# zjwzcx/A-2D-LiDAR-based-SLAM-System-for-Wheeled-Mobile-Robots

Measured on AMD Instinct MI355X. Metric: scans/sec (360-beam ICP + 0.05 m grid update), higher is better.
Workload: dtype f64; 1 GPU; configs[1]: 1000-scan replay (every 5th message of a 10 Hz stream, seed 1), 360 beams, ICP(max_iter=30, tol=0.001) + 400x400@0.05m grid, f64 point buffers; 32 independent replays of the 1000-scan trajectory per step (one slam_replay_dev call: ranges [32, 1000, 360], a map per trajectory); point_buffers=f64, pipeline=0, lanes=2, grid_mode=1, grid_group=16, parallelism=1 trajectory per GPU (32 independent replays of it per step)

## Files before the change

a-2d-lidar-based-slam-system-for-wheeled-mobile-robots_amd/csrc/icp_kernels.hip:

```cpp
#include <hip/hip_fp16.h>
#include <hip/hip_runtime.h>

#include <type_traits>

#include "slam_internal.h"
#include "slam_stamps.h"

namespace slam {

#ifdef SLAM_STAMPS_ICP
__device__ unsigned long long g_polar_lanes[4];
hipError_t debug_polar_lanes(unsigned long long out[4], bool clear)
{
    hipError_t e = hipMemcpyFromSymbol(out, HIP_SYMBOL(g_polar_lanes), sizeof(unsigned long long) * 4);
    if (e == hipSuccess && clear) {
        const unsigned long long zero[4] = {0ull, 0ull, 0ull, 0ull};
        e = hipMemcpyToSymbol(HIP_SYMBOL(g_polar_lanes), zero, sizeof zero);
    }
    return e;
}
#endif

__device__ __forceinline__ double ld(const double *p, long i) { return p[i]; }
__device__ __forceinline__ double ld(const float *p, long i) { return (double)p[i]; }
__device__ __forceinline__ double ld(const __half *p, long i) { return (double)__half2float(p[i]); }
__device__ __forceinline__ void st(double *p, long i, double v) { p[i] = v; }
__device__ __forceinline__ void st(float *p, long i, double v) { p[i] = (float)v; }
__device__ __forceinline__ void st(__half *p, long i, double v)
{
    float f = (float)v;
    if ((double)f != v && v == v) {
// ... 284 lines not shown
constexpr int kPolarMaxFirst = 16;
constexpr int kPolarMaxListed = 48;
constexpr int kPolarProbe = 8;
constexpr bool kOnePass = true;
constexpr int kPolarTail = 4;

template <typename T> struct StoreSlack { static constexpr float ang = 2e-7f; };
template <> struct StoreSlack<float> { static constexpr float ang = 1e-6f; };
template <> struct StoreSlack<__half> { static constexpr float ang = 3e-3f; };

struct PolarGeo {
    float inv_db;
    float slack;
};

template <int UNROLL, bool PROBE>
__device__ __forceinline__ void nn_polar(const double2 *__restrict__ tarP, int n_tar, double sx, double sy, int seed,
                                         bool active, const PolarGeo &geo, int wmax, double &best_d2, int &best_j, bool &big,
                                         bool &amb, unsigned long long &ambm)
{
    const float fsx = (float)sx, fsy = (float)sy;
    const float rs2 = fsx * fsx + fsy * fsy;
    int lo, hi;
    auto window = [&](int j, int &wlo, int &whi) -> bool {
        const double2 ts = tarP[j];
        const double U = dist2(sx, sy, ts.x, ts.y);
        const float ftx = (float)ts.x, fty = (float)ts.y;
        const float x2 = ((float)U * 1.000002f + 1e-30f) * __builtin_amdgcn_rcpf(rs2 * 0.999998f);
        const bool small = x2 < 0.25f;
        const float x = __builtin_amdgcn_sqrtf(x2) * 1.000001f;
        const float alpha = x * (1.0f + 0.19f * x2) * 1.000002f + geo.slack;
        const float y = (ftx * fsy - fty * fsx) * __builtin_amdgcn_rcpf(ftx * fsx + fty * fsy);
        const float y3 = y * y * y * 0.33333334f;
        const float dhi = (y >= 0.0f ? y : y - y3) + 4e-6f;
// ... 37 lines not shown
        pb.start();
        pb.j = seed;
        scan(need ? max(seed - kPolarProbe, 0) : 1, need ? min(seed + kPolarProbe, n_tar - 1) : 0, pb);
        int lo1, hi1;
        const bool fits1 = window(pb.j, lo1, hi1) && need;
        lo = fits1 ? lo1 : lo;
        hi = fits1 ? hi1 : hi;
        fits = fits || fits1;
    }
    big = active && !fits;
    const bool go = active && !big;
    const int m0 = max(lo, 0), m1 = min(hi, n_tar - 1);
    Best b;
    b.start();
    const bool wraps = __any(go && ((hi >= n_tar - 2 && lo >= 1) || (lo <= 1 && hi <= n_tar - 2)));
    if (wraps) {
        const int e0 = hi >= n_tar - 2 ? min(hi - (n_tar - 1) + 1, m0 - 1) : -1;
        scan(go ? 0 : 1, go ? e0 : 0, b);
    }
    scan(go ? m0 : 1, go ? m1 : 0, b);
    if (wraps) {
        const int s2 = lo <= 1 ? max(n_tar - 1 + lo - 1, m1 + 1) : n_tar;
        scan(go ? s2 : 1, go ? n_tar - 1 : 0, b);
    }
    best_d2 = b.d2;
    best_j = b.j;
    amb = go && b.amb();
    ambm = b.ambm;
}

// ... 265 lines not shown
    PolarGeo pg;
    pg.inv_db = polar ? __fdividef(1.000002f, dmin) : 0.0f;
    pg.slack = StoreSlack<T>::ang;
    return pg;
}

struct NNTarget {
    const double2 *tarP;
    const double2 *tarB;
    const Box *boxes, *boxes4;
    int nblocks, n_tar;
    bool has_p;
    double2 *qlist;
    int *qseed;
    int cap;
    __device__ __forceinline__ double2 at(int j) const { return has_p ? tarP[j] : tarB[tslot(j)]; }
};
struct NNQuery {
    double d2;
    int j;
    int slot;
};
__device__ __forceinline__ double match_distance(double d2) { return (d2 < INFINITY) ? sqrt(d2) : 0.0; }

template <int UNROLL, int STRIDE, bool EXACT, typename Place, typename NoteBig>
__device__ __forceinline__ NNQuery nn_query(const NNTarget &t, const PolarGeo &pg, const double sx, const double sy, const int seed, const bool okq,
                                            const bool first, const bool listing, Place &&place, NoteBig &&note_big, unsigned long long &amb_mask)
{
    NNQuery h;
    h.slot = -1;
    if (EXACT) {
        const bool padded = STRIDE == kNNStride && !t.has_p;
        const NNHit e = nn_exact(padded ? t.tarB : t.tarP, padded, okq ? t.n_tar : 0, sx, sy);
        h.d2 = e.d2; h.j = e.j;
    } else if (pg.inv_db > 0.0f) {
        bool big, amb_lane;
        unsigned long long am;
        nn_polar<UNROLL, false>(t.tarP, t.n_tar, sx, sy, seed, okq, pg, listing ? kPolarMaxFirst : kPolarMax, h.d2, h.j, big, amb_lane, am);
        (void)amb_lane;
        amb_mask |= am;
        if (listing) {
            const unsigned long long bm = __ballot(big);
            if (bm != 0ull) {
                const int pos = place(bm) + (int)__builtin_amdgcn_mbcnt_hi((unsigned)(bm >> 32), __builtin_amdgcn_mbcnt_lo((unsigned)bm, 0u));
                if (big && pos < t.cap) {
                    h.slot = pos;
                    t.qlist[pos] = make_double2(sx, sy);
                    t.qseed[pos] = seed;
                    big = false;
                }
            }
        }
        note_big(big);
// ... 361 lines not shown
    }
    if (tid == 0) store_result(a, b, r, s);
    ISTAMP(5);
    ISTAMP_END(s.iters);
    lds_guard_check(guard, a.status);
    return !EXACT && (nwaves > 1 ? geo[5] != 0u : amb_mask != 0ull);
}

constexpr int kWaveQpt = 6;
constexpr int kWaveRound = 4 * 1024;
__host__ __device__ inline int icp_wave_points(int n_tar)
{
    const int whole = nn_blocks(n_tar) * kNNBlock, tail = n_tar + kPolarTail;
    return whole > tail ? whole : tail;
}
__host__ __device__ inline size_t icp_wave_lds_bytes(int n_tar, int cap)
{
    return (size_t)icp_wave_points(n_tar) * sizeof(double2) + (size_t)(nn_boxes_padded(n_tar) + nn_boxes4(n_tar)) * sizeof(Box) +
           (size_t)cap * (sizeof(double2) + sizeof(int));
}

__device__ __forceinline__ double sqrt_unscaled(double x)
{
    const double y = __builtin_amdgcn_rsq(x);
    double g = x * y, h = y * 0.5;
    const double r = fma(-h, g, 0.5);
    g = fma(g, r, g);
    h = fma(h, r, h);
    g = fma(fma(-g, g, x), h, g);
    return fma(fma(-g, g, x), h, g);
}
constexpr unsigned kSqrtLoHi = 0x10100000u, kSqrtHiHi = 0x58F00000u;
__device__ __forceinline__ double match_distance_wave(double d2)
{
    const bool in = (unsigned)__double2hiint(d2) - kSqrtLoHi < kSqrtHiHi - kSqrtLoHi;
    if (__any(!in)) return match_distance(d2);
    return sqrt_unscaled(d2);
}

template <typename T, bool EXACT>
__device__ __forceinline__ bool icp_pair_wave(const IcpArgs &a, const int b, char *smem)
{
    constexpr int QPT = kWaveQpt;
    const int n_src = a.n_src, n_tar = a.n_tar, nblocks = nn_blocks(n_tar), lane = threadIdx.x;
    double2 *tarP = reinterpret_cast<double2 *>(smem);
    Box *boxes = reinterpret_cast<Box *>(tarP + icp_wave_points(n_tar));
    Box *boxes4 = boxes + nn_boxes_padded(n_tar);
    double2 *qlist = reinterpret_cast<double2 *>(boxes4 + nn_boxes4(n_tar));
    int *qseed = reinterpret_cast<int *>(qlist + a.team_cap);
    char *guard = reinterpret_cast<char *>(qseed + a.team_cap);
    lds_guard_fill(guard);

    const PairClouds<T> pc = pair_clouds<T>(a, b);
    const NNTarget nt{tarP, tarP, boxes, boxes4, nblocks, n_tar, true, qlist, qseed, a.team_cap};

    double sx[QPT], sy[QPT];
    int seed[QPT];
    bool src_differs = false;
    {
        const double2 p0 = pc.source(0, true);
#pragma unroll
        for (int q = 0; q < QPT; ++q) {
            const int i = lane + q * kWave;
            const double2 pt = pc.source(i, i < n_src);
            sx[q] = pt.x; sy[q] = pt.y;
            seed[q] = min(i, n_tar - 1);
            src_differs |= i < n_src && !(pt.x == p0.x && pt.y == p0.y);
        }
    }
// ... 69 lines not shown
                add_centred(w, sx[q], sy[q], c.ax, c.ay, m.x, m.y, c.bx, c.by);
            }
        }
        lanes4(wave_reduce4(w, ls), w);
        s.ca0x = c.ax; s.ca0y = c.ay;
        advance(rigid_from_w(c, w[0], w[1], w[2], w[3], tar_collapsed || src_collapsed, lane), c.bx, c.by, sx, sy, s);
        return converged(s, a.tol);
    };
    auto iteration = [&]() __attribute__((always_inline)) -> bool {
        double u[8] = {0, 0, 0, 0, 0, 0, 0, 0};
        SameMatch same{0.0, 0.0, false, false};
#pragma unroll
        for (int q = 0; q < QPT; ++q) {
            if (q * kWave >= n_src) continue;
            const bool okq = lane + q * kWave < n_src;
            const NNQuery h = nn_query<4, kNNBlock, EXACT>(nt, pg, sx[q], sy[q], seed[q], okq, false, false, place, no_note, amb_mask);
            seed[q] = h.j;
            const double2 m = tarP[h.j];
            same.step(q, okq, h.j, m.x, m.y);
            if (okq) add_one_pass(u, sx[q], sy[q], m.x, m.y, match_distance_wave(h.d2), s.pcx, s.pcy);
        }
        const OnePass o = one_pass_totals(wave_reduce8(u, ls), dn, s);
        advance(rigid_from_w(o.c, o.A, 0.0, o.B, 0.0, !same.wave_differs() || src_collapsed, lane), o.c.bx, o.c.by, sx, sy, s);
        return converged(s, a.tol);
    };
    if (a.max_iter > 0 && !first_iteration())
        for (int it = 1; it < a.max_iter; ++it)
            if (iteration()) break;

    Rigid2 r;
    if (s.iters > 0) {
        double u[4] = {0, 0, 0, 0};
#pragma unroll
        for (int q = 0; q < QPT; ++q) {
            if (q * kWave >= n_src) continue;
            const int i = lane + q * kWave;
            if (i < n_src) {
                const double2 o = pc.source(i, true);
                add_final(u, sx[q], sy[q], s.pcx, s.pcy, o.x, o.y, s.ca0x, s.ca0y);
            }
        }
        r = final_transform(wave_reduce4(u, ls), dn, s, src_collapsed, lane);
    } else {
// ... 22 lines not shown
    for (size_t i = (size_t)blockIdx.x * blockDim.x + threadIdx.x; i < n16; i += (size_t)gridDim.x * blockDim.x) p[i] = make_uint4(0u, 0u, 0u, 0u);
    if (blockIdx.x == 0 && threadIdx.x < ((a.zero_bytes & 15) >> 2)) static_cast<unsigned *>(a.zero_ptr)[(n16 << 2) + threadIdx.x] = 0u;
}

template <typename T, int QPT, int UNROLL>
__global__ void __launch_bounds__(1024) k_icp(IcpArgs a)
{
    extern __shared__ __attribute__((aligned(16))) char smem[];
    icp_clear_on_the_way(a);
    if (icp_pair<T, QPT, UNROLL, false>(a, blockIdx.x, smem)) {
        __syncthreads();
        icp_pair<T, QPT, 2, true>(a, blockIdx.x, smem);
    }
}

template <typename T>
__global__ void __launch_bounds__(kWave) __attribute__((amdgpu_waves_per_eu(4))) k_icp(IcpArgs a)
{
    extern __shared__ __attribute__((aligned(16))) char smem[];
    icp_clear_on_the_way(a);
    if (icp_pair_wave<T, false>(a, blockIdx.x, smem)) {
        wave_sync();
        icp_pair_wave<T, true>(a, blockIdx.x, smem);
    }
}

static inline int icp_block(int n_src, int qpt)
{
    int per = (n_src + qpt - 1) / qpt;
    int blk = ((per + kWave - 1) / kWave) * kWave;
    return blk < kWave ? kWave : blk;
}

template <typename T>
static hipError_t launch_icp_t(const IcpArgs &a_in, hipStream_t s)
{
    IcpArgs a = a_in;
    int qpt = (a.n_src + 1023) / 1024;
    const long waves_at_two = (long)a.B * ((a.n_src + 127) / 128);
    int pref = a.qpt_pref > 0 ? a.qpt_pref : (a.batch_invariant ? 2 : waves_at_two >= 7500 ? 3 : 2);
    if ((a.B > 64 || a.batch_invariant) && qpt < pref && a.n_src > 64 * pref) qpt = pref;
    if (qpt > 4) qpt = 8;
    {
        const int cap = (a.ranges && a.team_mode == 0) ? ((a.n_src + 3) / 4 + 15) / 16 * 16 : 0;
        const size_t lds = icp_wave_lds_bytes(a.n_tar, cap) + kLdsGuard;
        const bool fits = a.n_src <= kWave * kWaveQpt && lds <= 64 * 1024;
        const bool full = !a.batch_invariant && pref == 3 && a.B >= 4 * kWaveRound && a.n_src > kWave * 3 && a.ranges && lds <= 10 * 1024;
        if (fits && (a.one_wave == 1 || (a.one_wave < 0 && full))) {
            a.team_cap = cap;
            SLAM_LAUNCH((k_icp<T>), dim3(a.B), dim3(kWave), lds, s, a);
            return hipGetLastError();
        }
    }
    const int block = icp_block(a.n_src, qpt);
    const size_t lds_base = nn_lds_bytes(a.n_tar) + icp_red_bytes(block / kWave) + kIcpExtraLds + kLdsGuard;
    a.polar_copy = (a.ranges && lds_base + icp_polar_bytes(a.n_tar) <= 160 * 1024) ? 1 : 0;
    size_t lds = lds_base + (a.polar_copy ? icp_polar_bytes(a.n_tar) : 0);
    a.team_cap = 0;
    if (a.polar_copy && a.team_mode == 0) {
        long cap = ((a.n_src + 1) / 2 + 15) / 16 * 16;
        const long room = ((long)160 * 1024 - (long)lds) / (long)(sizeof(double2) + sizeof(int));
        cap = cap < room ? cap : room / 16 * 16;
        a.team_cap = cap > 0 ? (int)cap : 0;
    }
    lds += (size_t)a.team_cap * (sizeof(double2) + sizeof(int));
// ... 307 lines not shown
```

a-2d-lidar-based-slam-system-for-wheeled-mobile-robots_amd/csrc/slam_abi.hip:

```cpp
#include <hip/hip_runtime.h>

#include <algorithm>
#include <cmath>
#include <cstdarg>
#include <cstdio>
#include <cstring>
#include <string>
#include <initializer_list>
#include <mutex>
#include <utility>
#include <vector>

#include "slam_internal.h"
#include "slam_stamps.h"

using namespace slam;

namespace {

thread_local std::string g_err;

int fail(int code, const char *fmt, ...)
{
    char buf[512];
// ... 57 lines not shown
    Arena tiles;
    char *pinned = nullptr;
    size_t pinned_cap = 0;
    int *status = nullptr;
    bool timing = false;
    unsigned timing_mask = ~0u;
    std::vector<hipEvent_t> pool;
    std::vector<Pending> pending;
    double ms[SLAM_K_COUNT] = {0};
    int64_t launches[SLAM_K_COUNT] = {0};
    int grid_mode = 1;
    int grid_group = 0;
    int grid_split = -1;
    int icp_qpt = 0;
    int replay_reset = 0;
    int icp_one_wave = -1;
    int icp_team = 0;
    int pipeline = 0;
    hipStream_t gstream = nullptr;
    hipStream_t cstream = nullptr;
    hipEvent_t ev_fork = nullptr, ev_join = nullptr, ev_icp = nullptr, ev_pose = nullptr;
    hipEvent_t ev_cast[2] = {nullptr, nullptr};
    const void *cast_poses[2] = {nullptr, nullptr};
    const void *cast_T[2] = {nullptr, nullptr};
    double *pipe_T[2] = {nullptr, nullptr};
    size_t pipe_T_bytes = 0;
    int cast_pos = 0;
    bool gdirty = false;
    bool mgrid = false;
    int particle_chunks = 0;
// ... 526 lines not shown
    return check_status_sync(c);
}

struct OptionRange {
    const char *name;
    bool (*ok)(double);
    const char *msg;
};
static const OptionRange kOptionRanges[] = {
    {"grid_mode", [](double v) { return v == 0 || v == 1 || v == 2 || v == 3 || v == 4; }, "grid_mode is 0..4"},
    {"grid_group", [](double v) { return v >= 0 && v <= 64; }, "grid_group in [0, 64]"},
    {"grid_split", [](double v) { return v == -1 || v == 0 || v == 1; }, "grid_split is -1, 0 or 1"},
    {"replay_reset", [](double v) { return v == 0 || v == 1; }, "replay_reset is 0 or 1"},
    {"icp_team", [](double v) { return v == 0 || v == 1; }, "icp_team is 0 or 1"},
    {"icp_one_wave", [](double v) { return v == -1 || v == 0 || v == 1; }, "icp_one_wave is -1, 0 or 1"},
    {"particle_chunks", [](double v) { return v >= 0 && v <= 64 && v == (int)v; }, "particle_chunks in [0, 64]"},
    {"icp_qpt", [](double v) { return v >= 0 && v <= 3; }, "icp_qpt in [0, 3]"},
    {"pipeline", [](double v) { return v == 0 || v == 1; }, "pipeline is 0 or 1"},
};

int slam_set_option(slam_ctx *c, const char *name, double value)
{
    REQUIRE(name, "null name");
    const OptionRange *opt = nullptr;
    for (const OptionRange &o : kOptionRanges)
        if (!strcmp(name, o.name)) opt = &o;
    if (!opt) return fail(SLAM_ERR_INVALID, "unknown option %s", name);
    REQUIRE(opt->ok(value), opt->msg);
    TRY(use(c));
    if (!strcmp(name, "grid_mode")) c->grid_mode = (int)value;
    else if (!strcmp(name, "grid_group")) c->grid_group = (int)value;
    else if (!strcmp(name, "grid_split")) c->grid_split = (int)value;
    else if (!strcmp(name, "replay_reset")) c->replay_reset = (int)value;
    else if (!strcmp(name, "icp_team")) c->icp_team = (int)value;
    else if (!strcmp(name, "icp_one_wave")) c->icp_one_wave = (int)value;
    else if (!strcmp(name, "particle_chunks")) { TRY(join_particles(c)); c->particle_chunks = (int)value; }
    else if (!strcmp(name, "icp_qpt")) c->icp_qpt = (int)value;
    else if (!strcmp(name, "pipeline")) {
        TRY(join_from_grid(c));
        if (value == 1 && !c->gstream) {
            HIPCHK(hipStreamCreateWithFlags(&c->gstream, hipStreamNonBlocking));
            HIPCHK(hipStreamCreateWithFlags(&c->cstream, hipStreamNonBlocking));
            for (hipEvent_t *e : {&c->ev_fork, &c->ev_join, &c->ev_icp, &c->ev_pose, &c->ev_cast[0], &c->ev_cast[1]})
                HIPCHK(hipEventCreateWithFlags(e, hipEventDisableTiming));
        }
        if (value == 0 && c->pipeline) HIPCHK(hipStreamSynchronize(c->gstream));
        c->pipeline = (int)value;
        c->cast_poses[0] = c->cast_poses[1] = nullptr;
        c->cast_T[0] = c->cast_T[1] = nullptr;
    }
// ... 36 lines not shown
    }
    return SLAM_OK;
}

#if defined(SLAM_STAMPS) || defined(SLAM_STAMPS_ICP)
int slam_debug_read(slam_ctx *c, void *out256, int clear)
{
    TRY(use(c));
    HIPCHK(hipStreamSynchronize(c->stream));
    HIPCHK(hipMemcpy(out256, c->status, 256, hipMemcpyDeviceToHost));
    if (clear) HIPCHK(hipMemset(reinterpret_cast<char *>(c->status) + 32, 0, 224));
    return SLAM_OK;
}
#endif
#ifdef SLAM_STAMPS_ICP
int slam_debug_lanes(slam_ctx *c, unsigned long long *out4, int clear)
{
    TRY(use(c));
    HIPCHK(hipStreamSynchronize(c->stream));
    HIPCHK(slam::debug_polar_lanes(out4, clear != 0));
    return SLAM_OK;
}
#endif
#ifdef SLAM_STAMPS
int slam_debug_records(slam_ctx *c, void *out, int max_records)
{
    TRY(use(c));
    HIPCHK(hipStreamSynchronize(c->stream));
    const int n = max_records < kStampRecords ? max_records : kStampRecords;
    HIPCHK(hipMemcpy(out, reinterpret_cast<char *>(c->status) + 256, (size_t)n * 32, hipMemcpyDeviceToHost));
    return SLAM_OK;
}
#endif


// ... 107 lines not shown

int slam_icp_batch_dev(slam_ctx *c, const void *tar, const void *src, int B, int n_tar, int n_src, int dtype,
                       int tar_shared, int src_shared, const double *prior, int max_iter, double tol, double *T_out,
                       int32_t *iters_out, double *mean_err_out)
{
    TRY(use(c));
    TRY(check_icp_batch(__func__, tar, src, B, n_tar, n_src, dtype, max_iter, T_out));
    IcpArgs a;
    a.tar = tar; a.src = src; a.prior = prior;
    a.ranges = nullptr; a.cos_t = a.sin_t = nullptr; a.tar_scan_stride = a.src_scan_stride = 0;
    a.tar_stride = tar_shared ? 0 : 2L * n_tar;
    a.src_stride = src_shared ? 0 : 2L * n_src;
    a.ppt = 0;
    a.B = B; a.n_tar = n_tar; a.n_src = n_src; a.max_iter = max_iter; a.tol = tol;
    a.T_out = T_out; a.iters_out = iters_out; a.err_out = mean_err_out;
    a.status = c->status; a.qpt_pref = c->icp_qpt; a.team_mode = c->icp_team; a.one_wave = c->icp_one_wave;
    Timed t(c, SLAM_K_ICP);
    HIPCHK(launch_icp(a, dtype, c->stream));
    return SLAM_OK;
}

int slam_icp_batch(slam_ctx *c, const void *tar, const void *src, int B, int n_tar, int n_src, int dtype, int tar_shared,
                   int src_shared, const double *prior, int max_iter, double tol, double *T_out, int32_t *iters_out,
                   double *mean_err_out)
{
    TRY(use(c));
    TRY(check_icp_batch(__func__, tar, src, B, n_tar, n_src, dtype, max_iter, T_out));
    const size_t ds = dtype_size(dtype);
    char *d_t, *d_s; double *d_p, *d_T, *d_e; int32_t *d_i;
    Staging s(c);
    s.in(d_t, static_cast<const char *>(tar), (size_t)(tar_shared ? 1 : B) * 2 * n_tar * ds)
// ... 419 lines not shown
        for (int k = 0; k < 2; ++k)
            if (c->cast_poses[k] && (c->cast_poses[k] == poses_out || c->cast_T[k] == T)) {
                HIPCHK(hipStreamWaitEvent(c->stream, c->ev_cast[k], 0));
                HIPCHK(hipStreamWaitEvent(c->cstream, c->ev_cast[k], 0));
                c->cast_poses[k] = c->cast_T[k] = nullptr;
            }
    {
        IcpArgs a;
        a.tar = a.src = nullptr; a.prior = nullptr;
        a.ranges = ranges; a.cos_t = cos_t; a.sin_t = sin_t;
        a.tar_scan_stride = a.src_scan_stride = n;
        a.tar_stride = a.src_stride = 0;
        a.ppt = n_scan - 1;
        a.B = (int)pairs; a.n_tar = n; a.n_src = n; a.max_iter = max_iter; a.tol = tol;
        a.T_out = T; a.iters_out = iters_out; a.err_out = nullptr;
        a.status = c->status; a.qpt_pref = c->icp_qpt; a.team_mode = c->icp_team; a.one_wave = c->icp_one_wave;
        if (grid && c->replay_reset) {
            if (piped || grid->pmap_live) {
                TRY(slam_grid_reset(c, grid));
            } else {
                a.zero_ptr = grid->d.pass; a.zero_bytes = grid->state_bytes;
                grid->pristine = true;
            }
        }
        Timed t(c, SLAM_K_ICP);
        HIPCHK(launch_icp(a, dtype, c->stream));
    }
    if (!piped) {
        {
            Timed t(c, SLAM_K_COMPOSE);
            HIPCHK(launch_pose_compose(T, pose0, L, n_scan - 1, poses_out, c->stream));
// ... 90 lines not shown
        TRY(arena_reserve(c, c->scratch, need));
        heading_cs = carve<double>(c->scratch, (size_t)P * 2);
        grid->pristine = false;
    }
    for (int k = 0; k < chunks; ++k) {
        const int p0 = (int)((long)P * k / chunks), pc = (int)((long)P * (k + 1) / chunks) - p0;
        {
            IcpArgs a;
            a.tar = a.src = nullptr; a.prior = prior ? prior + 6 * (size_t)p0 : nullptr;
            a.ranges = ranges2; a.cos_t = cos_t; a.sin_t = sin_t;
            a.tar_scan_stride = a.src_scan_stride = 0;
            a.tar_stride = a.src_stride = 0;
            a.ppt = 0;
            a.B = pc; a.n_tar = n; a.n_src = n; a.max_iter = max_iter; a.tol = tol;
            a.T_out = T_out + 9 * (size_t)p0; a.iters_out = iters_out ? iters_out + p0 : nullptr; a.err_out = nullptr;
            a.status = c->status; a.team_mode = c->icp_team; a.one_wave = c->icp_one_wave;
            a.qpt_pref = c->icp_qpt > 0 ? c->icp_qpt : (P >= 2500 ? 3 : 0);
            Timed t(c, SLAM_K_ICP, nullptr, k == 0);
            HIPCHK(launch_icp(a, dtype, c->stream));
        }
        {
            Timed t(c, SLAM_K_COMPOSE, nullptr, k == 0);
            HIPCHK(launch_pose_compose(T_out + 9 * (size_t)p0, pose_prev + 3 * (size_t)p0, pc, 1, poses_out + 3 * (size_t)p0, c->stream,
                                       prior ? prior + 6 * (size_t)p0 : nullptr, heading_cs ? heading_cs + 2 * (size_t)p0 : nullptr));
        }
        if (grid) {
            hipStream_t st = c->stream;
            if (chunks > 1) {
                HIPCHK(hipEventRecord(c->pev_pose[k], c->stream));
                HIPCHK(hipStreamWaitEvent(c->pstream, c->pev_pose[k], 0));
                st = c->pstream;
// ... 490 lines not shown
    {
        LandmarkArgs a{ranges, cos_t, sin_t, (long)S, n, range_threshold, radius_max_th, lm_cap, cnt, ovf, ids, means, z, nullptr, c->status};
        HIPCHK(launch_landmarks(a, c->stream));
        HIPCHK(launch_node_keep(cnt, L, n_scan, kept_out, kept_count_out, c->stream));
        HIPCHK(launch_node_gather(ranges, kept_out, kept_count_out, L, n_scan, n, kr, c->stream));
    }
    {
        IcpArgs a;
        a.tar = a.src = nullptr; a.prior = nullptr;
        a.ranges = kr; a.cos_t = cos_t; a.sin_t = sin_t;
        a.tar_scan_stride = a.src_scan_stride = n;
        a.tar_stride = a.src_stride = 0;
        a.ppt = n_scan - 1;
        a.B = (int)pairs; a.n_tar = n; a.n_src = n; a.max_iter = max_iter; a.tol = tol;
        a.T_out = T; a.iters_out = iters_out; a.err_out = nullptr;
        a.status = c->status; a.qpt_pref = c->icp_qpt; a.team_mode = c->icp_team; a.one_wave = c->icp_one_wave;
        a.batch_invariant = 1;
        Timed t(c, SLAM_K_ICP);
        HIPCHK(launch_icp(a, dtype, c->stream));
    }
    {
        EkfArgs a{};
        a.B = L; a.steps_max = n_scan - 1; a.max_lm = max_lm;
        a.x0 = pose0; a.steps = kept_count_out; a.steps_bias = 1; a.T = T; a.z = z;
        a.kept = kept_out; a.lm_count = cnt; a.lm_overflow = ovf; a.lm_cap = lm_cap;
        a.x_out = x_final_out; a.P_out = P_final_out; a.nlm_hist = nlm_out; a.status_out = status_out;
        a.x_hist = xest_out; a.cast_poses = grid ? cast_poses : nullptr; a.status = c->status;
        HIPCHK(launch_ekf_lm(a, c->stream));
    }
    if (grid) {
        TRY(grid_on_main(c));
// ... 56 lines not shown
    TRY(use(c));
    TRY(check_loc_replay(__func__, ranges, S, n_scan, n, stream_of_traj, ox, oy, obs_off, M, K, L, cos_t, sin_t, angle_min,
                         angle_increment, max_iter, xest_out, xodom_out, P_final_out, status_out));
    const size_t Lz = (size_t)L, pairs = (size_t)S * (2 * (size_t)n_scan - 1);
    TRY(arena_reserve(c, c->scratch, align_up(pairs * 4 * n * 8) + align_up(pairs * 72) + 2 * align_up(Lz * 2 * n * 8) +
                                         align_up(Lz * 72) + align_up(Lz * 4) + align_up(Lz * kLocStateDoubles * 8) + 4096));
    double *pair_pts = carve<double>(c->scratch, pairs * 4 * n), *T_stream = carve<double>(c->scratch, pairs * 9);
    double *tar = carve<double>(c->scratch, Lz * 2 * n), *src = carve<double>(c->scratch, Lz * 2 * n);
    double *T_step = carve<double>(c->scratch, Lz * 9);
    int32_t *it_step = carve<int32_t>(c->scratch, Lz);
    double *state = carve<double>(c->scratch, Lz * kLocStateDoubles);
    REQUIRE(pair_pts && T_stream && tar && src && T_step && it_step && state, "internal: workspace");
    IcpArgs icp;
    icp.prior = nullptr; icp.ranges = nullptr; icp.cos_t = icp.sin_t = nullptr; icp.tar_scan_stride = icp.src_scan_stride = 0;
    icp.ppt = 0; icp.n_tar = n; icp.n_src = n; icp.max_iter = max_iter; icp.tol = tol; icp.err_out = nullptr;
    icp.status = c->status; icp.qpt_pref = c->icp_qpt; icp.team_mode = c->icp_team; icp.one_wave = c->icp_one_wave;
    icp.batch_invariant = 1;
    {
        HIPCHK(launch_loc_stream_pairs(ranges, cos_t, sin_t, S, n_scan, n, pair_pts, c->stream));
        icp.tar = pair_pts; icp.src = pair_pts + 2 * (size_t)n; icp.tar_stride = icp.src_stride = 4L * n;
        icp.B = (int)pairs; icp.T_out = T_stream; icp.iters_out = nullptr;
        Timed t(c, SLAM_K_ICP);
        HIPCHK(launch_icp(icp, SLAM_F64, c->stream));
    }
    LocArgs a{};
    a.L = L; a.S = S; a.M = M; a.n = n; a.n_scan = n_scan;
    a.ranges = ranges; a.stream_of_traj = stream_of_traj; a.map_of_traj = map_of_traj;
    a.ox = ox; a.oy = oy; a.obs_off = obs_off; a.K = K; a.pose0 = pose0; a.cos_t = cos_t; a.sin_t = sin_t;
    a.angle_min = angle_min; a.angle_increment = angle_increment;
    a.T_stream = T_stream; a.T_step = T_step; a.iters_step = it_step; a.state = state; a.tar_pts = tar; a.src_pts = src;
    a.xest_out = xest_out; a.xodom_out = xodom_out; a.P_final_out = P_final_out; a.status_out = status_out;
// ... 49 lines not shown
```

a-2d-lidar-based-slam-system-for-wheeled-mobile-robots_amd/csrc/slam_internal.h:

```cpp
#pragma once

#include <hip/hip_runtime.h>
#include <stdint.h>
#include <string.h>

#include "slam_hip.h"

#include <hip/hip_ext.h>

namespace slam {

struct LaunchTimer {
    void *self;
    bool (*next)(void *self, hipEvent_t *e0, hipEvent_t *e1);
};
extern thread_local LaunchTimer g_launch_timer;
inline bool launch_events(hipEvent_t *e0, hipEvent_t *e1)
{
    return g_launch_timer.self && g_launch_timer.next(g_launch_timer.self, e0, e1);
}

#define SLAM_LAUNCH(kernel, grid, block, shmem, stream, ...)                                                          \
    do {                                                                                                              \
        hipEvent_t e0_ = nullptr, e1_ = nullptr;                                                                      \
// ... 41 lines not shown
    long tar_stride, src_stride;
    int ppt;
    int B, n_tar, n_src, max_iter;
    double tol;
    double *T_out;
    int32_t *iters_out;
    double *err_out;
    int *status = nullptr;
    int qpt_pref = 0;
    void *zero_ptr = nullptr;
    size_t zero_bytes = 0;
    int polar_copy = 0;
    int team_cap = 0;
    int team_mode = 0;
    int one_wave = -1;
    int batch_invariant = 0;
};

hipError_t launch_icp(const IcpArgs &a, int dtype, hipStream_t s);
hipError_t launch_nn(const void *src, const void *tar, int B, int n_src, int n_tar, int dtype, double *dist,
                     int32_t *idx, hipStream_t s);
hipError_t launch_kabsch(const double *src, const double *tar, int B, int n, double *T_out, hipStream_t s);
hipError_t launch_scan_to_points(const float *ranges, const double *cos_t, const double *sin_t, long total,
                                 int n, int clip_inf, int dtype, void *pts, hipStream_t s);
hipError_t launch_pose_compose(const double *T, const double *pose0, int L, int n, double *poses, hipStream_t s,
                               const double *prior = nullptr, double *heading_cs = nullptr);

#ifdef SLAM_STAMPS_ICP
hipError_t debug_polar_lanes(unsigned long long out[4], bool clear);
#endif

constexpr int kMaxHitLevels = 8;
constexpr int kVisitSlots = 256;
constexpr int kVisitStride = 8;
#if defined(__HIPCC__)
__device__ __forceinline__ unsigned long long *visit_slot(unsigned long long *visits)
{
    return visits + (size_t)((blockIdx.x + blockIdx.y * 131u) & (unsigned)(kVisitSlots - 1)) * kVisitStride;
}
#endif

struct GridDev {
    int G, xw, yw;
    double scale, off_x, off_y;
// ... 171 lines not shown
```

a-2d-lidar-based-slam-system-for-wheeled-mobile-robots_amd/csrc/slam_stamps.h:

```cpp
#pragma once

#ifdef SLAM_STAMPS
constexpr int kStampRecords = 32768;
#define STAMP_DECL unsigned long long st_t0 = __builtin_amdgcn_s_memtime(), st_first = st_t0; unsigned st_rec[5] = {0u, 0u, 0u, 0u, 0u}; unsigned st_real = (unsigned)__builtin_amdgcn_s_memrealtime()
#define STAMP(k)                                                                                         \
    do {                                                                                                 \
        if (threadIdx.x == 0) {                                                                          \
            unsigned long long t_ = __builtin_amdgcn_s_memtime();                                        \
            atomicAdd(reinterpret_cast<unsigned long long *>(g.status + 8) + (k), t_ - st_t0);           \
            st_rec[(k) < 5 ? (k) : 4] += (unsigned)(t_ - st_t0);                                         \
            st_t0 = t_;                                                                                  \
        }                                                                                                \
    } while (0)
#define STAMP_END(k)                                                                                     \
    do {                                                                                                 \
        if (threadIdx.x == 0) {                                                                          \
            unsigned long long t_ = __builtin_amdgcn_s_memtime();                                        \
            atomicAdd(reinterpret_cast<unsigned long long *>(g.status + 8) + (k), t_ - st_first);        \
            const unsigned long long id_ = atomicAdd(reinterpret_cast<unsigned long long *>(g.status + 8) + (k) + 1, 1ull); \
            if (id_ < (unsigned long long)kStampRecords) {                                               \
                unsigned *r_ = reinterpret_cast<unsigned *>(g.status) + 64 + 8 * id_;                    \
                for (int q_ = 0; q_ < 5; ++q_) r_[q_] = st_rec[q_];                                      \
                r_[5] = (unsigned)(t_ - st_first); r_[6] = blockIdx.x | (blockIdx.y << 16); r_[7] = st_real; \
            }                                                                                            \
// ... 8 lines not shown
#define STAMP_WAVE_COUNT(k, v)                        \
    do {                                                                                                 \
        if ((threadIdx.x & 63) == 0) atomicAdd(reinterpret_cast<unsigned long long *>(g.status + 8) + (k), (unsigned long long)(v)); \
    } while (0)
#else
#define STAMP_DECL
#define STAMP(k)
#define STAMP_END(k)
#define STAMP_SYNC()
#define STAMP_COUNT(k, v)
#define STAMP_WAVE_COUNT(k, v)
#define STAMP_VAL(v)
#endif

#if defined(SLAM_STAMPS_ICP) && SLAM_STAMPS_ICP != 3
extern __device__ unsigned long long g_polar_lanes[4];
#define ISTAMP_SCAN(first, own, trips, per_trip)                                                          \
    do {                                                                                                 \
        unsigned o_ = (unsigned)(own);                                                                   \
        for (int off_ = 32; off_ > 0; off_ >>= 1) o_ += __shfl_xor(o_, off_);                            \
        if ((threadIdx.x & 63) == 0) {                                                                   \
            atomicAdd(&g_polar_lanes[(first) ? 0 : 2], (unsigned long long)o_);                          \
            atomicAdd(&g_polar_lanes[(first) ? 1 : 3], (unsigned long long)(trips) * (per_trip) * 64ull); \
        }                                                                                                \
    } while (0)
#else
#define ISTAMP_SCAN(first, own, trips, per_trip)
#endif

#ifdef SLAM_STAMPS_ICP
#define ISTAMP_DECL unsigned long long st_t0 = __builtin_amdgcn_s_memtime(), st_first = st_t0, st_acc[15] = {0, 0, 0, 0, 0, 0, 0, 0, 0, 0, 0, 0, 0, 0, 0}, st_big[4] = {0, 0, 0, 0}, st_real = __builtin_amdgcn_s_memrealtime()
#define ISTAMP(k)                                                                                        \
    do {                                                                                                 \
        unsigned long long t_ = __builtin_amdgcn_s_memtime();                                            \
        st_acc[k] += t_ - st_t0;                                                                         \
        st_t0 = t_;                                                                                      \
    } while (0)
#if SLAM_STAMPS_ICP == 2
#define ISTAMP_END(iters)                                                                                \
    do {                                                                                                 \
        if (threadIdx.x == 0) {                                                                          \
            unsigned long long *c_ = reinterpret_cast<unsigned long long *>(a.status + 8);              \
// ... 41 lines not shown
```

Measured before the change: 18.17 million scans/s.

## Add f32 prefilter for polar nearest-neighbour scan with certified fallback to f64

Before the ICP iterations, the target cloud is staged into LDS as a float2 image, reusing the query-list region. The polar-window NN search then runs a float32 key-min scan that tracks the best and runner-up candidates. If an error bound shows the f32 winner is unambiguous for every active lane in the wave, the f64 distance is computed only for that winner. Otherwise the wave falls back to the original f64 scan. This aims to cut costly f64 arithmetic in the inner NN loop, at the cost of a staging pass, extra LDS, and duplicated work whenever the fallback triggers.

```diff
diff --git a/a-2d-lidar-based-slam-system-for-wheeled-mobile-robots_amd/csrc/icp_kernels.hip b/a-2d-lidar-based-slam-system-for-wheeled-mobile-robots_amd/csrc/icp_kernels.hip
--- a/a-2d-lidar-based-slam-system-for-wheeled-mobile-robots_amd/csrc/icp_kernels.hip
+++ b/a-2d-lidar-based-slam-system-for-wheeled-mobile-robots_amd/csrc/icp_kernels.hip
@@ -9,12 +9,12 @@
 namespace slam {
 
 #ifdef SLAM_STAMPS_ICP
-__device__ unsigned long long g_polar_lanes[4];
-hipError_t debug_polar_lanes(unsigned long long out[4], bool clear)
-{
-    hipError_t e = hipMemcpyFromSymbol(out, HIP_SYMBOL(g_polar_lanes), sizeof(unsigned long long) * 4);
+__device__ unsigned long long g_polar_lanes[6];
+hipError_t debug_polar_lanes(unsigned long long out[6], bool clear)
+{
+    hipError_t e = hipMemcpyFromSymbol(out, HIP_SYMBOL(g_polar_lanes), sizeof(unsigned long long) * 6);
     if (e == hipSuccess && clear) {
-        const unsigned long long zero[4] = {0ull, 0ull, 0ull, 0ull};
+        const unsigned long long zero[6] = {0ull, 0ull, 0ull, 0ull, 0ull, 0ull};
         e = hipMemcpyToSymbol(HIP_SYMBOL(g_polar_lanes), zero, sizeof zero);
     }
     return e;
@@ -329,10 +329,57 @@
     float slack;
 };
 
-template <int UNROLL, bool PROBE>
+struct F32Image {
+    const float2 *img;
+    float tmax;
+};
+constexpr unsigned kF32Inf = 0x7f800000u;
+
+struct F32Best {
+    unsigned m, r;
+    int kb;
+    __device__ __forceinline__ void start() { m = r = kF32Inf; kb = 0; }
+    __device__ __forceinline__ void take(unsigned k)
+    {
+        r = max(min(m, k), min(max(m, k), r));
+        m = min(m, k);
+    }
+    __device__ __forceinline__ int index() const { return kb + (int)(m & 3u); }
+    __device__ __forceinline__ bool settled(float fsx, float fsy, float tmax) const
+    {
+        const float km = __uint_as_float(m), kr = __uint_as_float(r);
+        const float a = __builtin_amdgcn_sqrtf(km) * 1.000002f;
+        const float ef = (fabsf(fsx) + fabsf(fsy) + tmax) * (0x1p-23f * 1.00001f);
+        const float b = a + 2.0f * ef;
+        return b * b * 1.000002f + 1e-30f < fminf(kr * 0.999998f, 1e30f);
+    }
+};
+
+__device__ __forceinline__ unsigned f32_key(float fsx, float fsy, float2 t, unsigned place)
+{
+    const float dx = fsx - t.x, dy = fsy - t.y;
+    return (__float_as_uint(fmaf(dy, dy, dx * dx)) & ~3u) | place;
+}
+
+__device__ __forceinline__ void scan32(const float2 *__restrict__ img, int n_tar, float fsx, float fsy, int a0, int a1, F32Best &b)
+{
+    for (int k = a0; __any(k <= a1); k += 4) {
+        const int kc = k <= a1 ? k : n_tar;
+        const float2 *t = img + kc;
+        const float2 t0 = t[0], t1 = t[1], t2 = t[2], t3 = t[3];
+        const unsigned before = b.m;
+        b.take(f32_key(fsx, fsy, t0, 0u));
+        b.take(f32_key(fsx, fsy, t1, 1u));
+        b.take(f32_key(fsx, fsy, t2, 2u));
+        b.take(f32_key(fsx, fsy, t3, 3u));
+        b.kb = b.m < before ? kc : b.kb;
+    }
+}
+
+template <int UNROLL, bool PROBE, bool F32 = false>
 __device__ __forceinline__ void nn_polar(const double2 *__restrict__ tarP, int n_tar, double sx, double sy, int seed,
                                          bool active, const PolarGeo &geo, int wmax, double &best_d2, int &best_j, bool &big,
-                                         bool &amb, unsigned long long &ambm)
+                                         bool &amb, unsigned long long &ambm, const F32Image f32 = F32Image{nullptr, 0.0f})
 {
     const float fsx = (float)sx, fsy = (float)sy;
     const float rs2 = fsx * fsx + fsy * fsy;
@@ -400,6 +447,30 @@
     Best b;
     b.start();
     const bool wraps = __any(go && ((hi >= n_tar - 2 && lo >= 1) || (lo <= 1 && hi <= n_tar - 2)));
+    if (F32) {
+        F32Best fb;
+        fb.start();
+        if (wraps) {
+            const int e0 = hi >= n_tar - 2 ? min(hi - (n_tar - 1) + 1, m0 - 1) : -1;
+            scan32(f32.img, n_tar, fsx, fsy, go ? 0 : 1, go ? e0 : 0, fb);
+        }
+        scan32(f32.img, n_tar, fsx, fsy, go ? m0 : 1, go ? m1 : 0, fb);
+        if (wraps) {
+            const int s2 = lo <= 1 ? max(n_tar - 1 + lo - 1, m1 + 1) : n_tar;
+            scan32(f32.img, n_tar, fsx, fsy, go ? s2 : 1, go ? n_tar - 1 : 0, fb);
+        }
+        const bool fell_back = __any(go && !fb.settled(fsx, fsy, f32.tmax));
+        ISTAMP_F32(fell_back);
+        if (!fell_back) {
+            const int j = fb.index();
+            const double2 t = tarP[j];
+            best_d2 = go ? dist2(sx, sy, t.x, t.y) : INFINITY;
+            best_j = j;
+            amb = false;
+            ambm = 0ull;
+            return;
+        }
+    }
     if (wraps) {
         const int e0 = hi >= n_tar - 2 ? min(hi - (n_tar - 1) + 1, m0 - 1) : -1;
         scan(go ? 0 : 1, go ? e0 : 0, b);
@@ -695,6 +766,7 @@
     double2 *qlist;
     int *qseed;
     int cap;
+    F32Image f32 = F32Image{nullptr, 0.0f};
     __device__ __forceinline__ double2 at(int j) const { return has_p ? tarP[j] : tarB[tslot(j)]; }
 };
 struct NNQuery {
@@ -704,7 +776,7 @@
 };
 __device__ __forceinline__ double match_distance(double d2) { return (d2 < INFINITY) ? sqrt(d2) : 0.0; }
 
-template <int UNROLL, int STRIDE, bool EXACT, typename Place, typename NoteBig>
+template <int UNROLL, int STRIDE, bool EXACT, bool F32 = false, typename Place, typename NoteBig>
 __device__ __forceinline__ NNQuery nn_query(const NNTarget &t, const PolarGeo &pg, const double sx, const double sy, const int seed, const bool okq,
                                             const bool first, const bool listing, Place &&place, NoteBig &&note_big, unsigned long long &amb_mask)
 {
@@ -717,7 +789,7 @@
     } else if (pg.inv_db > 0.0f) {
         bool big, amb_lane;
         unsigned long long am;
-        nn_polar<UNROLL, false>(t.tarP, t.n_tar, sx, sy, seed, okq, pg, listing ? kPolarMaxFirst : kPolarMax, h.d2, h.j, big, amb_lane, am);
+        nn_polar<UNROLL, false, F32>(t.tarP, t.n_tar, sx, sy, seed, okq, pg, listing ? kPolarMaxFirst : kPolarMax, h.d2, h.j, big, amb_lane, am, t.f32);
         (void)amb_lane;
         amb_mask |= am;
         if (listing) {
@@ -1109,10 +1181,11 @@
     const int whole = nn_blocks(n_tar) * kNNBlock, tail = n_tar + kPolarTail;
     return whole > tail ? whole : tail;
 }
-__host__ __device__ inline size_t icp_wave_lds_bytes(int n_tar, int cap)
-{
+__host__ __device__ inline size_t icp_wave_lds_bytes(int n_tar, int cap, bool f32)
+{
+    const size_t list = (size_t)cap * (sizeof(double2) + sizeof(int)), image = f32 ? (size_t)icp_wave_points(n_tar) * sizeof(float2) : 0;
     return (size_t)icp_wave_points(n_tar) * sizeof(double2) + (size_t)(nn_boxes_padded(n_tar) + nn_boxes4(n_tar)) * sizeof(Box) +
-           (size_t)cap * (sizeof(double2) + sizeof(int));
+           (list > image ? list : image);
 }
 
 __device__ __forceinline__ double sqrt_unscaled(double x)
@@ -1133,7 +1206,7 @@
     return sqrt_unscaled(d2);
 }
 
-template <typename T, bool EXACT>
+template <typename T, bool EXACT, bool F32>
 __device__ __forceinline__ bool icp_pair_wave(const IcpArgs &a, const int b, char *smem)
 {
     constexpr int QPT = kWaveQpt;
@@ -1143,11 +1216,12 @@
     Box *boxes4 = boxes + nn_boxes_padded(n_tar);
     double2 *qlist = reinterpret_cast<double2 *>(boxes4 + nn_boxes4(n_tar));
     int *qseed = reinterpret_cast<int *>(qlist + a.team_cap);
-    char *guard = reinterpret_cast<char *>(qseed + a.team_cap);
+    float2 *tarF = reinterpret_cast<float2 *>(qlist);
+    char *guard = smem + icp_wave_lds_bytes(n_tar, a.team_cap, F32);
     lds_guard_fill(guard);
 
     const PairClouds<T> pc = pair_clouds<T>(a, b);
-    const NNTarget nt{tarP, tarP, boxes, boxes4, nblocks, n_tar, true, qlist, qseed, a.team_cap};
+    NNTarget nt{tarP, tarP, boxes, boxes4, nblocks, n_tar, true, qlist, qseed, a.team_cap};
 
     double sx[QPT], sy[QPT];
     int seed[QPT];
@@ -1247,7 +1321,7 @@
         for (int q = 0; q < QPT; ++q) {
             if (q * kWave >= n_src) continue;
             const bool okq = lane + q * kWave < n_src;
-            const NNQuery h = nn_query<4, kNNBlock, EXACT>(nt, pg, sx[q], sy[q], seed[q], okq, false, false, place, no_note, amb_mask);
+            const NNQuery h = nn_query<4, kNNBlock, EXACT, F32 && !EXACT>(nt, pg, sx[q], sy[q], seed[q], okq, false, false, place, no_note, amb_mask);
             seed[q] = h.j;
             const double2 m = tarP[h.j];
             same.step(q, okq, h.j, m.x, m.y);
@@ -1257,9 +1331,25 @@
         advance(rigid_from_w(o.c, o.A, 0.0, o.B, 0.0, !same.wave_differs() || src_collapsed, lane), o.c.bx, o.c.by, sx, sy, s);
         return converged(s, a.tol);
     };
-    if (a.max_iter > 0 && !first_iteration())
+    auto stage_f32 = [&]() __attribute__((always_inline)) {
+        wave_sync();
+        float tm = 0.0f;
+        for (int j = lane; j < icp_wave_points(n_tar); j += kWave) {
+            const double2 t = tarP[j];
+            const float fx = t.x == t.x ? (float)t.x : INFINITY, fy = t.y == t.y ? (float)t.y : INFINITY;
+            tarF[j] = make_float2(fx, fy);
+            if (t.x == t.x && t.y == t.y) tm = fmaxf(tm, fabsf(fx) + fabsf(fy));
+        }
+#pragma unroll
+        for (int off = 32; off > 0; off >>= 1) tm = fmaxf(tm, __shfl_xor(tm, off));
+        nt.f32 = F32Image{tarF, __uint_as_float((unsigned)__builtin_amdgcn_readfirstlane((int)__float_as_uint(tm * 1.000001f)))};
+        wave_sync();
+    };
+    if (a.max_iter > 0 && !first_iteration()) {
+        if (F32 && !EXACT && pg.inv_db > 0.0f && a.max_iter > 1) stage_f32();
         for (int it = 1; it < a.max_iter; ++it)
             if (iteration()) break;
+    }
 
     Rigid2 r;
     if (s.iters > 0) {
@@ -1312,14 +1402,14 @@
     }
 }
 
-template <typename T>
+template <typename T, bool F32>
 __global__ void __launch_bounds__(kWave) __attribute__((amdgpu_waves_per_eu(4))) k_icp(IcpArgs a)
 {
     extern __shared__ __attribute__((aligned(16))) char smem[];
     icp_clear_on_the_way(a);
-    if (icp_pair_wave<T, false>(a, blockIdx.x, smem)) {
+    if (icp_pair_wave<T, false, F32>(a, blockIdx.x, smem)) {
         wave_sync();
-        icp_pair_wave<T, true>(a, blockIdx.x, smem);
+        icp_pair_wave<T, true, F32>(a, blockIdx.x, smem);
     }
 }
 
@@ -1341,12 +1431,14 @@
     if (qpt > 4) qpt = 8;
     {
         const int cap = (a.ranges && a.team_mode == 0) ? ((a.n_src + 3) / 4 + 15) / 16 * 16 : 0;
-        const size_t lds = icp_wave_lds_bytes(a.n_tar, cap) + kLdsGuard;
+        const bool f32 = a.f32_filter != 0 && a.ranges;
+        const size_t lds = icp_wave_lds_bytes(a.n_tar, cap, f32) + kLdsGuard;
         const bool fits = a.n_src <= kWave * kWaveQpt && lds <= 64 * 1024;
-        const bool full = !a.batch_invariant && pref == 3 && a.B >= 4 * kWaveRound && a.n_src > kWave * 3 && a.ranges && lds <= 10 * 1024;
+        const bool full = !a.batch_invariant && pref == 3 && a.B >= 4 * kWaveRound && a.n_src > kWave * 3 && a.ranges && lds - kLdsGuard <= 10 * 1024;
         if (fits && (a.one_wave == 1 || (a.one_wave < 0 && full))) {
             a.team_cap = cap;
-            SLAM_LAUNCH((k_icp<T>), dim3(a.B), dim3(kWave), lds, s, a);
+            if (f32) SLAM_LAUNCH((k_icp<T, true>), dim3(a.B), dim3(kWave), lds, s, a);
+            else SLAM_LAUNCH((k_icp<T, false>), dim3(a.B), dim3(kWave), lds, s, a);
             return hipGetLastError();
         }
     }
diff --git a/a-2d-lidar-based-slam-system-for-wheeled-mobile-robots_amd/csrc/slam_abi.hip b/a-2d-lidar-based-slam-system-for-wheeled-mobile-robots_amd/csrc/slam_abi.hip
--- a/a-2d-lidar-based-slam-system-for-wheeled-mobile-robots_amd/csrc/slam_abi.hip
+++ b/a-2d-lidar-based-slam-system-for-wheeled-mobile-robots_amd/csrc/slam_abi.hip
@@ -95,6 +95,7 @@
     int grid_split = -1;
     int icp_qpt = 0;
     int replay_reset = 0;
+    int icp_f32_filter = -1;
     int icp_one_wave = -1;
     int icp_team = 0;
     int pipeline = 0;
@@ -651,6 +652,7 @@
     {"replay_reset", [](double v) { return v == 0 || v == 1; }, "replay_reset is 0 or 1"},
     {"icp_team", [](double v) { return v == 0 || v == 1; }, "icp_team is 0 or 1"},
     {"icp_one_wave", [](double v) { return v == -1 || v == 0 || v == 1; }, "icp_one_wave is -1, 0 or 1"},
+    {"icp_f32_filter", [](double v) { return v == -1 || v == 0 || v == 1; }, "icp_f32_filter is -1, 0 or 1"},
     {"particle_chunks", [](double v) { return v >= 0 && v <= 64 && v == (int)v; }, "particle_chunks in [0, 64]"},
     {"icp_qpt", [](double v) { return v >= 0 && v <= 3; }, "icp_qpt in [0, 3]"},
     {"pipeline", [](double v) { return v == 0 || v == 1; }, "pipeline is 0 or 1"},
@@ -671,6 +673,7 @@
     else if (!strcmp(name, "replay_reset")) c->replay_reset = (int)value;
     else if (!strcmp(name, "icp_team")) c->icp_team = (int)value;
     else if (!strcmp(name, "icp_one_wave")) c->icp_one_wave = (int)value;
+    else if (!strcmp(name, "icp_f32_filter")) c->icp_f32_filter = (int)value;
     else if (!strcmp(name, "particle_chunks")) { TRY(join_particles(c)); c->particle_chunks = (int)value; }
     else if (!strcmp(name, "icp_qpt")) c->icp_qpt = (int)value;
     else if (!strcmp(name, "pipeline")) {
@@ -737,11 +740,11 @@
 }
 #endif
 #ifdef SLAM_STAMPS_ICP
-int slam_debug_lanes(slam_ctx *c, unsigned long long *out4, int clear)
+int slam_debug_lanes(slam_ctx *c, unsigned long long *out6, int clear)
 {
     TRY(use(c));
     HIPCHK(hipStreamSynchronize(c->stream));
-    HIPCHK(slam::debug_polar_lanes(out4, clear != 0));
+    HIPCHK(slam::debug_polar_lanes(out6, clear != 0));
     return SLAM_OK;
 }
 #endif
@@ -879,7 +882,7 @@
     a.ppt = 0;
     a.B = B; a.n_tar = n_tar; a.n_src = n_src; a.max_iter = max_iter; a.tol = tol;
     a.T_out = T_out; a.iters_out = iters_out; a.err_out = mean_err_out;
-    a.status = c->status; a.qpt_pref = c->icp_qpt; a.team_mode = c->icp_team; a.one_wave = c->icp_one_wave;
+    a.status = c->status; a.qpt_pref = c->icp_qpt; a.team_mode = c->icp_team; a.one_wave = c->icp_one_wave; a.f32_filter = c->icp_f32_filter;
     Timed t(c, SLAM_K_ICP);
     HIPCHK(launch_icp(a, dtype, c->stream));
     return SLAM_OK;
@@ -1329,7 +1332,7 @@
         a.ppt = n_scan - 1;
         a.B = (int)pairs; a.n_tar = n; a.n_src = n; a.max_iter = max_iter; a.tol = tol;
         a.T_out = T; a.iters_out = iters_out; a.err_out = nullptr;
-        a.status = c->status; a.qpt_pref = c->icp_qpt; a.team_mode = c->icp_team; a.one_wave = c->icp_one_wave;
+        a.status = c->status; a.qpt_pref = c->icp_qpt; a.team_mode = c->icp_team; a.one_wave = c->icp_one_wave; a.f32_filter = c->icp_f32_filter;
         if (grid && c->replay_reset) {
             if (piped || grid->pmap_live) {
                 TRY(slam_grid_reset(c, grid));
@@ -1450,7 +1453,7 @@
             a.ppt = 0;
             a.B = pc; a.n_tar = n; a.n_src = n; a.max_iter = max_iter; a.tol = tol;
             a.T_out = T_out + 9 * (size_t)p0; a.iters_out = iters_out ? iters_out + p0 : nullptr; a.err_out = nullptr;
-            a.status = c->status; a.team_mode = c->icp_team; a.one_wave = c->icp_one_wave;
+            a.status = c->status; a.team_mode = c->icp_team; a.one_wave = c->icp_one_wave; a.f32_filter = c->icp_f32_filter;
             a.qpt_pref = c->icp_qpt > 0 ? c->icp_qpt : (P >= 2500 ? 3 : 0);
             Timed t(c, SLAM_K_ICP, nullptr, k == 0);
             HIPCHK(launch_icp(a, dtype, c->stream));
@@ -1971,7 +1974,7 @@
         a.ppt = n_scan - 1;
         a.B = (int)pairs; a.n_tar = n; a.n_src = n; a.max_iter = max_iter; a.tol = tol;
         a.T_out = T; a.iters_out = iters_out; a.err_out = nullptr;
-        a.status = c->status; a.qpt_pref = c->icp_qpt; a.team_mode = c->icp_team; a.one_wave = c->icp_one_wave;
+        a.status = c->status; a.qpt_pref = c->icp_qpt; a.team_mode = c->icp_team; a.one_wave = c->icp_one_wave; a.f32_filter = c->icp_f32_filter;
         a.batch_invariant = 1;
         Timed t(c, SLAM_K_ICP);
         HIPCHK(launch_icp(a, dtype, c->stream));
@@ -2058,7 +2061,7 @@
     IcpArgs icp;
     icp.prior = nullptr; icp.ranges = nullptr; icp.cos_t = icp.sin_t = nullptr; icp.tar_scan_stride = icp.src_scan_stride = 0;
     icp.ppt = 0; icp.n_tar = n; icp.n_src = n; icp.max_iter = max_iter; icp.tol = tol; icp.err_out = nullptr;
-    icp.status = c->status; icp.qpt_pref = c->icp_qpt; icp.team_mode = c->icp_team; icp.one_wave = c->icp_one_wave;
+    icp.status = c->status; icp.qpt_pref = c->icp_qpt; icp.team_mode = c->icp_team; icp.one_wave = c->icp_one_wave; icp.f32_filter = c->icp_f32_filter;
     icp.batch_invariant = 1;
     {
         HIPCHK(launch_loc_stream_pairs(ranges, cos_t, sin_t, S, n_scan, n, pair_pts, c->stream));
diff --git a/a-2d-lidar-based-slam-system-for-wheeled-mobile-robots_amd/csrc/slam_internal.h b/a-2d-lidar-based-slam-system-for-wheeled-mobile-robots_amd/csrc/slam_internal.h
--- a/a-2d-lidar-based-slam-system-for-wheeled-mobile-robots_amd/csrc/slam_internal.h
+++ b/a-2d-lidar-based-slam-system-for-wheeled-mobile-robots_amd/csrc/slam_internal.h
@@ -79,6 +79,7 @@
     int team_cap = 0;
     int team_mode = 0;
     int one_wave = -1;
+    int f32_filter = -1;
     int batch_invariant = 0;
 };
 
@@ -92,7 +93,7 @@
                                const double *prior = nullptr, double *heading_cs = nullptr);
 
 #ifdef SLAM_STAMPS_ICP
-hipError_t debug_polar_lanes(unsigned long long out[4], bool clear);
+hipError_t debug_polar_lanes(unsigned long long out[6], bool clear);
 #endif
 
 constexpr int kMaxHitLevels = 8;
diff --git a/a-2d-lidar-based-slam-system-for-wheeled-mobile-robots_amd/csrc/slam_stamps.h b/a-2d-lidar-based-slam-system-for-wheeled-mobile-robots_amd/csrc/slam_stamps.h
--- a/a-2d-lidar-based-slam-system-for-wheeled-mobile-robots_amd/csrc/slam_stamps.h
+++ b/a-2d-lidar-based-slam-system-for-wheeled-mobile-robots_amd/csrc/slam_stamps.h
@@ -46,7 +46,14 @@
 #endif
 
 #if defined(SLAM_STAMPS_ICP) && SLAM_STAMPS_ICP != 3
-extern __device__ unsigned long long g_polar_lanes[4];
+extern __device__ unsigned long long g_polar_lanes[6];
+#define ISTAMP_F32(fell_back)                                                                            \
+    do {                                                                                                 \
+        if ((threadIdx.x & 63) == 0) {                                                                   \
+            atomicAdd(&g_polar_lanes[4], 1ull);                                                          \
+            if (fell_back) atomicAdd(&g_polar_lanes[5], 1ull);                                           \
+        }                                                                                                \
+    } while (0)
 #define ISTAMP_SCAN(first, own, trips, per_trip)                                                          \
     do {                                                                                                 \
         unsigned o_ = (unsigned)(own);                                                                   \
@@ -58,6 +65,7 @@
     } while (0)
 #else
 #define ISTAMP_SCAN(first, own, trips, per_trip)
+#define ISTAMP_F32(fell_back)
 #endif
 
 #ifdef SLAM_STAMPS_ICP
```

Result: faster. 18.63 million scans/s (median of 6 runs) (+2.5%).
